# tensorflow/adanet

Measured on NVIDIA H100. Metric: candidate-train examples/sec per AdaNet iteration, higher is better.
Workload: dtype f32

## Files before the change

### adanet_b200/csrc/planes.cu

```cuda
#include <cuda.h>
#include <cudaTypedefs.h>

#include <stdlib.h>
#include <string.h>

#include <algorithm>
#include <atomic>
#include <mutex>
#include <string>
#include <unordered_map>
#include <vector>

#include "dense_simt.cuh"
#include "planes.cuh"
#include "wgmma.cuh"

namespace adn {
namespace pl {

static constexpr int BM = 128, BN = 64;
static constexpr int STAGES = 3;
static constexpr int A_TILE = BM * 128;
static constexpr int B_TILE = BN * 128;
static constexpr int STAGE_BYTES = 2 * A_TILE + 2 * B_TILE;
// ... 5 lines not shown
static_assert(128 * (PRODUCER_REGS + EPI_REGS) + 128 * CONSUMERS * CONSUMER_REGS <= 65536, "register file");
static_assert(PRODUCER_REGS < 65536 / NUM_THREADS && EPI_REGS > 65536 / NUM_THREADS &&
              CONSUMER_REGS > 65536 / NUM_THREADS, "setmaxnreg.dec / .inc");
static constexpr int ACC_BUFS = 2;
static constexpr int ACC_TILE_FLOATS = BM * BN;
static constexpr int ACC_BYTES = ACC_BUFS * ACC_TILE_FLOATS * 4;
static constexpr int EPI_STAGE_FLOATS = 32 * 16;
static constexpr int EPI_BYTES = EPI_WARPS * 2 * EPI_STAGE_FLOATS * 4;
static constexpr int BAR_BYTES = 256;
static constexpr int SMEM_BYTES = 1024 + STAGES * STAGE_BYTES + ACC_BYTES + EPI_BYTES + BAR_BYTES;
static_assert(SMEM_BYTES <= 232448, "shared memory per block");
static constexpr int MAX_SPLITS = 64;

template <int FMT> struct Fmt;
template <> struct Fmt<FMT_TF32> {
  static constexpr int BK = 32;
  static constexpr int CHUNK = 4;
};
template <> struct Fmt<FMT_F16> {
  static constexpr int BK = 64;
  static constexpr int CHUNK = 2;
};

enum { EPI_BIAS_ACT = 0, EPI_MASK = 1, EPI_PARTIAL = 2 };

struct GemmParams {
  int M, N;
  int tiles_m, tiles_n, splits;
  int tiles;
  float inv_tiles, inv_tiles_n, inv_tiles_m;
  int total_kb;
  int kb_per_split;
  int a_mn, b_mn;
  int out_planes;
  int m_fastest;
  void* out;
  void* out_lo;
  int ldc;
  int out_nb32;
  int out_tma;
  const float* bias;
  int act;
  uint32_t* out_bits;
  const uint32_t* mask_bits;
  float* colsum_part;
  int colsum_ld;
  float out_mul;
  unsigned int* ovf;
  uint32_t drop_thresh;
// ... 375 lines not shown
        }
        if (rsub == 0) {
          float* cp = g.colsum_part + (size_t)(mrow0 >> 5) * g.colsum_ld + col;
#pragma unroll
          for (int k = 0; k < 4; ++k)
            if (col + k < g.colsum_ld) cp[k] = cs[k];
        }
      }
    }
    __syncwarp();
  }
#undef ADN_SWZ
}

static constexpr int MAX_GROUP = 8;

struct alignas(64) Problem {
  CUtensorMap a_hi, a_lo, b_hi, b_lo;
  CUtensorMap o_hi, o_lo;
  GemmParams g;
  int item0;
  int pad_[3];
};
struct alignas(64) Group {
  Problem p[MAX_GROUP];
  int n;
  int total_items;
};

__device__ __forceinline__ int find_problem(const Group& grp, int cur, int item, int& next0) {
  while (item >= next0) {
    ++cur;
    next0 = (cur + 1 < grp.n) ? grp.p[cur + 1].item0 : 0x7fffffff;
  }
  return cur;
}
__device__ __forceinline__ int first_next0(const Group& grp) { return grp.n > 1 ? grp.p[1].item0 : 0x7fffffff; }

struct EpiItem {
  int p;
  Item it;
  uint32_t mw0, mw1;
  uint32_t drop_step;
};
template <int EPI>
__device__ __forceinline__ EpiItem epi_fetch(const Group& grp, int& cur, int& next0, int item, int tile_row) {
  EpiItem e;
  cur = find_problem(grp, cur, item, next0);
  e.p = cur;
  const GemmParams& g = grp.p[cur].g;
  e.it = decode_item(g, item - grp.p[cur].item0);
  e.mw0 = e.mw1 = 0xffffffffu;
  if (EPI == EPI_MASK && g.mask_bits) {
    const int my_row = e.it.m0 + tile_row, kbo = e.it.n0 >> 5;
    const bool row_ok = my_row < g.M;
    e.mw0 = (row_ok && kbo < g.out_nb32) ? __ldg(g.mask_bits + (size_t)kbo * g.M + my_row) : 0u;
    e.mw1 = (row_ok && kbo + 1 < g.out_nb32) ? __ldg(g.mask_bits + (size_t)(kbo + 1) * g.M + my_row) : 0u;
  }
  e.drop_step = (EPI == EPI_BIAS_ACT && g.drop_thresh != 0u) ? (uint32_t)(*g.drop_step) : 0u;
  return e;
}

template <int R> __device__ __forceinline__ void setmaxnreg_inc() { asm volatile("setmaxnreg.inc.sync.aligned.u32 %0;" ::"n"(R)); }
template <int R> __device__ __forceinline__ void setmaxnreg_dec() { asm volatile("setmaxnreg.dec.sync.aligned.u32 %0;" ::"n"(R)); }

__device__ __forceinline__ int acc_off(int row, int col) {
  return row * BN + ((((col >> 2) ^ row) & 7) | ((col >> 2) & 8)) * 4 + (col & 3);
}

template <int FMT>
__device__ __forceinline__ void fold_chunk(float (&acc)[32], const float (&H)[32], const float (&S)[32]) {
#pragma unroll
  for (int j = 0; j < 32; ++j) acc[j] += H[j];
  if (FMT == FMT_F16) {
#pragma unroll
    for (int j = 0; j < 32; ++j) acc[j] = fmaf(S[j], 1.0f / 2048.0f, acc[j]);
  } else {
#pragma unroll
    for (int j = 0; j < 32; ++j) acc[j] += S[j];
  }
}

template <int A_MN, int B_MN>
__device__ __forceinline__ void f16_kblock(uint32_t st, int wgi, float (&H)[32], float (&S)[32], bool first) {
  const uint32_t a_hi = st + (uint32_t)wgi * 8192u, a_lo = a_hi + A_TILE;
  const uint32_t b_hi = st + 2 * A_TILE, b_lo = b_hi + B_TILE;
  constexpr uint32_t a_step = A_MN ? 2048u : 32u, b_step = B_MN ? 2048u : 32u;
#pragma unroll
  for (int k = 0; k < 4; ++k) {
    const uint32_t sd = (first && k == 0) ? 0u : 1u;
    const uint64_t dah = wg::desc_sw128(a_hi + k * a_step), dal = wg::desc_sw128(a_lo + k * a_step);
    const uint64_t dbh = wg::desc_sw128(b_hi + k * b_step), dbl = wg::desc_sw128(b_lo + k * b_step);
    wg::mma_f16_n64<A_MN, B_MN>(H, dah, dbh, sd);
    wg::mma_f16_n64<A_MN, B_MN>(S, dah, dbl, sd);
    wg::mma_f16_n64<A_MN, B_MN>(S, dal, dbh, 1u);
  }
}

__device__ __forceinline__ uint32_t sw128_off(int r, int c) {
  return (uint32_t)(r * 128 + ((((c >> 4) ^ r) & 7) << 4) + (c & 15));
}
template <int MN>
// ... 13 lines not shown
  const uint8_t* bh = st + 2 * A_TILE;
  const uint8_t* bl = bh + B_TILE;
  const int gid = lane >> 2, tq = lane & 3;
#pragma unroll
  for (int ks = 0; ks < 4; ++ks) {
    uint32_t fa_h[4], fa_l[4];
#pragma unroll
    for (int e = 0; e < 4; ++e) {
      const uint32_t o = tf32_off<A_MN>(arow0 + gid + 8 * (e & 1), 8 * ks + tq + 4 * (e >> 1));
      fa_h[e] = *reinterpret_cast<const uint32_t*>(ah + o);
      fa_l[e] = *reinterpret_cast<const uint32_t*>(al + o);
    }
#pragma unroll
    for (int j = 0; j < 8; ++j) {
      const uint32_t o0 = tf32_off<B_MN>(8 * j + gid, 8 * ks + tq), o1 = tf32_off<B_MN>(8 * j + gid, 8 * ks + tq + 4);
      const uint32_t bh0 = *reinterpret_cast<const uint32_t*>(bh + o0), bh1 = *reinterpret_cast<const uint32_t*>(bh + o1);
      const uint32_t bl0 = *reinterpret_cast<const uint32_t*>(bl + o0), bl1 = *reinterpret_cast<const uint32_t*>(bl + o1);
      mma_tf32_16x8(&H[4 * j], fa_h, bh0, bh1);
      mma_tf32_16x8(&S[4 * j], fa_h, bl0, bl1);
      mma_tf32_16x8(&S[4 * j], fa_l, bh0, bh1);
    }
  }
}
template <int FMT, int EPI>
__global__ void __launch_bounds__(NUM_THREADS, 1)
pl_gemm_kernel(const __grid_constant__ Group grp) {
  constexpr int BK = Fmt<FMT>::BK;
  constexpr int CHUNK = Fmt<FMT>::CHUNK;
  constexpr int A_MN = EPI == EPI_PARTIAL, B_MN = EPI != EPI_MASK;
  extern __shared__ uint8_t smem_raw[];
  uint8_t* smem = reinterpret_cast<uint8_t*>((reinterpret_cast<uintptr_t>(smem_raw) + 1023) & ~(uintptr_t)1023);
  float* acc_stage = reinterpret_cast<float*>(smem + STAGES * STAGE_BYTES);
  float* epi_stage = reinterpret_cast<float*>(smem + STAGES * STAGE_BYTES + ACC_BYTES);
  uint64_t* bars = reinterpret_cast<uint64_t*>(smem + STAGES * STAGE_BYTES + ACC_BYTES + EPI_BYTES);
  uint64_t* full_bar = bars;
  uint64_t* empty_bar = bars + STAGES;
  uint64_t* tile_full = bars + 2 * STAGES;
  uint64_t* tile_empty = tile_full + ACC_BUFS;

  const int warp = __shfl_sync(0xffffffffu, threadIdx.x >> 5, 0);
  const int lane = threadIdx.x & 31;
  const int n_items = grp.total_items;

  if (threadIdx.x == 0) {
    for (int s = 0; s < STAGES; ++s) {
      mbar_init(smem_u32(&full_bar[s]), 1);
      mbar_init(smem_u32(&empty_bar[s]), CONSUMER_WARPS);
    }
    for (int b = 0; b < ACC_BUFS; ++b) {
      mbar_init(smem_u32(&tile_full[b]), 128 * CONSUMERS);
      mbar_init(smem_u32(&tile_empty[b]), 32 * EPI_WARPS);
    }
    asm volatile("fence.mbarrier_init.release.cluster;" ::: "memory");
  }
  if (warp == 1 && lane < grp.n) {
    tma_prefetch_desc(&grp.p[lane].a_hi);
    tma_prefetch_desc(&grp.p[lane].a_lo);
    tma_prefetch_desc(&grp.p[lane].b_hi);
    tma_prefetch_desc(&grp.p[lane].b_lo);
  }
  __syncthreads();

  if (warp < 4) {
    setmaxnreg_dec<PRODUCER_REGS>();
    if (warp == 0 && lane == 0) {
      uint32_t s = 0, ph = 0;
      int cur = 0, next0 = first_next0(grp);
      const uint32_t smem0 = smem_u32(smem);
      for (int item = blockIdx.x; item < n_items; item += gridDim.x) {
        cur = find_problem(grp, cur, item, next0);
        const Problem& pr = grp.p[cur];
        const GemmParams& g = pr.g;
        const Item it = decode_item(g, item - pr.item0);
        for (int kb = 0; kb < it.nkb; ++kb) {
          mbar_wait(smem_u32(&empty_bar[s]), ph ^ 1);
          const uint32_t fb = smem_u32(&full_bar[s]);
          mbar_expect_tx(fb, STAGE_BYTES);
          const uint32_t base = smem0 + s * STAGE_BYTES;
          const int kc = it.kb0 + kb;
          const int a1 = A_MN ? kc * BK : it.m0, a2 = A_MN ? (it.m0 / BK) : kc;
          const int b1 = B_MN ? kc * BK : it.n0, b2 = B_MN ? (it.n0 / BK) : kc;
          tma_load_3d(&pr.a_hi, fb, base, 0, a1, a2);
          tma_load_3d(&pr.a_lo, fb, base + A_TILE, 0, a1, a2);
          tma_load_3d(&pr.b_hi, fb, base + 2 * A_TILE, 0, b1, b2);
          tma_load_3d(&pr.b_lo, fb, base + 2 * A_TILE + B_TILE, 0, b1, b2);
          if (++s == STAGES) { s = 0; ph ^= 1; }
        }
      }
    }
    return;
  }

  if (warp >= 4 * (1 + CONSUMERS)) {
    setmaxnreg_inc<EPI_REGS>();
    const int ew = warp - 4 * (1 + CONSUMERS);
    float* stage = epi_stage + ew * 2 * EPI_STAGE_FLOATS;
    const int row = 32 * ew + lane;
    int cur = 0, next0 = first_next0(grp);
    EpiItem nx{};
    if ((int)blockIdx.x < n_items) nx = epi_fetch<EPI>(grp, cur, next0, blockIdx.x, row);
    uint32_t tcount = 0;
    for (int item = blockIdx.x; item < n_items; item += gridDim.x, ++tcount) {
      const EpiItem e = nx;
      if (item + (int)gridDim.x < n_items) nx = epi_fetch<EPI>(grp, cur, next0, item + gridDim.x, row);
      const GemmParams& g = grp.p[e.p].g;
      const Item& it = e.it;
      const uint32_t buf = tcount & 1u;
      mbar_wait(smem_u32(&tile_full[buf]), (tcount >> 1) & 1u);
      const float* tile = acc_stage + buf * ACC_TILE_FLOATS;
      const int mrow0 = it.m0 + 32 * ew;
      float* dense = reinterpret_cast<float*>(g.out);
      if (EPI == EPI_PARTIAL) dense += (size_t)it.split * g.M * g.N;
      const bool out_planes = g.out_planes != 0;
      const bool dense_vec = !out_planes && ((g.ldc & 3) == 0) && ((reinterpret_cast<uintptr_t>(dense) & 15) == 0);
      const int rows_ok = min(32, g.M - mrow0);
      const uint32_t mw0 = e.mw0, mw1 = e.mw1;
#pragma unroll 1
      for (int h = 0; h < 2; ++h) {
        const int cs = 32 * h;
        float acc[32];
#pragma unroll
        for (int q = 0; q < 8; ++q) {
          const float4 v = *reinterpret_cast<const float4*>(tile + acc_off(row, cs + 4 * q));
          acc[4 * q] = v.x; acc[4 * q + 1] = v.y; acc[4 * q + 2] = v.z; acc[4 * q + 3] = v.w;
        }
        if (h == 1) mbar_arrive(smem_u32(&tile_empty[buf]));
        const int ncol0 = it.n0 + cs;
        const uint32_t mw = h ? mw1 : mw0;
        if (FMT == FMT_F16 && !out_planes) {
          if (lane == 0) bulk_wait_read0();
          __syncwarp();
        }
        emit_slice<FMT, EPI>(g, out_planes, acc, mw, stage, lane, mrow0, ncol0, rows_ok, dense, dense_vec, true,
                             &grp.p[e.p].o_hi, &grp.p[e.p].o_lo, e.drop_step);
      }
    }
    if (FMT == FMT_F16 && lane == 0) bulk_wait0();
    return;
  }

  setmaxnreg_inc<CONSUMER_REGS>();
  const int wgi = warp / 4 - 1;
  const int wq = warp & 3;
  const int gid = lane >> 2, tq = lane & 3;
  const uint32_t smem0 = smem_u32(smem);
  uint32_t s = 0, ph = 0;
  int cur = 0, next0 = first_next0(grp);
  uint32_t tcount = 0;
  float H[32], S[32];
#pragma unroll
  for (int j = 0; j < 32; ++j) H[j] = S[j] = 0.f;
  for (int item = blockIdx.x; item < n_items; item += gridDim.x, ++tcount) {
    cur = find_problem(grp, cur, item, next0);
    const GemmParams& g = grp.p[cur].g;
    const Item it = decode_item(g, item - grp.p[cur].item0);
    float acc[32];
#pragma unroll
    for (int j = 0; j < 8; ++j)
#pragma unroll
      for (int e = 0; e < 4; ++e) {
        const int col = it.n0 + 8 * j + 2 * tq + (e & 1);
        acc[4 * j + e] = (EPI == EPI_BIAS_ACT && g.bias && col < g.N) ? __ldg(g.bias + col) : 0.f;
      }
    for (int kb = 0; kb < it.nkb; ++kb) {
      const bool first = (kb % CHUNK) == 0;
      const bool last = (kb % CHUNK) == CHUNK - 1 || kb == it.nkb - 1;
      mbar_wait(smem_u32(&full_bar[s]), ph);
      if (FMT == FMT_F16) {
        wg::fence_regs(H);
        wg::fence_regs(S);
        wg::fence();
        f16_kblock<A_MN, B_MN>(smem0 + s * STAGE_BYTES, wgi, H, S, first);
        wg::commit();
        wg::wait<0>();
        wg::fence_regs(H);
        wg::fence_regs(S);
      } else {
        if (first) {
#pragma unroll
          for (int j = 0; j < 32; ++j) H[j] = S[j] = 0.f;
        }
        tf32_kblock<A_MN, B_MN>(smem + s * STAGE_BYTES, 64 * wgi + 16 * wq, lane, H, S);
      }
      __syncwarp();
      if (lane == 0) mbar_arrive(smem_u32(&empty_bar[s]));
      if (++s == STAGES) { s = 0; ph ^= 1; }
      if (last) fold_chunk<FMT>(acc, H, S);
    }
    const uint32_t buf = tcount & 1u;
    mbar_wait(smem_u32(&tile_empty[buf]), ((tcount >> 1) & 1u) ^ 1u);
    float* tile = acc_stage + buf * ACC_TILE_FLOATS;
#pragma unroll
    for (int j = 0; j < 8; ++j) {
      const int row = 64 * wgi + 16 * wq + gid, col = 8 * j + 2 * tq;
      *reinterpret_cast<float2*>(tile + acc_off(row, col)) = make_float2(acc[4 * j], acc[4 * j + 1]);
      *reinterpret_cast<float2*>(tile + acc_off(row + 8, col)) = make_float2(acc[4 * j + 2], acc[4 * j + 3]);
    }
    mbar_arrive(smem_u32(&tile_full[buf]));
  }
}

template <int FMT>
__global__ void __launch_bounds__(256)
split_kernel(const float* __restrict__ src, void* __restrict__ hi_, void* __restrict__ lo_, uint32_t* __restrict__ bits,
             int rows, int cols, int nkb, float scale, unsigned int* ovf) {
  constexpr int BK = Fmt<FMT>::BK;
  const int vec_per_row = nkb * (BK / 4);
  const int64_t nvec = (int64_t)rows * vec_per_row;
  const int64_t nvec_pad = (nvec + 31) & ~(int64_t)31;
  const bool vec_src = ((cols & 3) == 0) && ((reinterpret_cast<uintptr_t>(src) & 15) == 0);
  bool over = false;
  for (int64_t i = (int64_t)blockIdx.x * blockDim.x + threadIdx.x; i < nvec_pad; i += (int64_t)gridDim.x * blockDim.x) {
    const bool live = i < nvec;
    const int r = live ? (int)(i / vec_per_row) : 0;
    const int c = live ? (int)(i % vec_per_row) * 4 : 0;
    float v[4] = {0.f, 0.f, 0.f, 0.f};
    if (live) {
      if (vec_src && c + 3 < cols) {
        float4 t = __ldg(reinterpret_cast<const float4*>(src + (size_t)r * cols + c));
        v[0] = t.x; v[1] = t.y; v[2] = t.z; v[3] = t.w;
      } else {
// ... 82 lines not shown
  ADN_CUDA(cudaStreamSynchronize(st));
  *out_host = (int)v;
  return ADN_OK;
}

int init() {
  static std::once_flag once;
  static int rc = ADN_OK;
  std::call_once(once, []() {
    void* fn = nullptr;
    cudaDriverEntryPointQueryResult q;
    cudaError_t e = cudaGetDriverEntryPoint("cuTensorMapEncodeTiled", &fn, cudaEnableDefault, &q);
    if (e != cudaSuccess || q != cudaDriverEntryPointSuccess || fn == nullptr) {
      (void)cudaGetLastError();
      rc = fail(ADN_ERR_CUDA, "pl::init: cuTensorMapEncodeTiled entry point unavailable");
      return;
    }
    g_encode = reinterpret_cast<PFN_cuTensorMapEncodeTiled>(fn);
    bool ok = true;
#define ADN_PL_ATTR(F, E) \
  ok = ok && (cudaFuncSetAttribute(pl_gemm_kernel<F, E>, cudaFuncAttributeMaxDynamicSharedMemorySize, SMEM_BYTES) == cudaSuccess)
    ADN_PL_ATTR(FMT_TF32, EPI_BIAS_ACT); ADN_PL_ATTR(FMT_TF32, EPI_MASK); ADN_PL_ATTR(FMT_TF32, EPI_PARTIAL);
    ADN_PL_ATTR(FMT_F16, EPI_BIAS_ACT); ADN_PL_ATTR(FMT_F16, EPI_MASK); ADN_PL_ATTR(FMT_F16, EPI_PARTIAL);
#undef ADN_PL_ATTR
    if (!ok) {
      (void)cudaGetLastError();
      rc = fail(ADN_ERR_CUDA, "pl::init: cudaFuncSetAttribute(smem=%d) failed", SMEM_BYTES);
      return;
    }
    void* addr = nullptr;
    if (cudaGetSymbolAddress(&addr, g_plane_overflow) != cudaSuccess || !addr) {
      (void)cudaGetLastError();
      rc = fail(ADN_ERR_CUDA, "pl::init: cudaGetSymbolAddress(g_plane_overflow) failed");
      return;
    }
    g_ovf_addr = reinterpret_cast<unsigned int*>(addr);
  });
  return rc;
}

int64_t planes_bytes_fmt(int fmt, int64_t rows, int64_t cols) { return planes_bytes(fmt, rows, cols); }

struct Operand {
  const void* hi;
  const void* lo;
  int64_t rows, nkb;
// ... 95 lines not shown
  GemmParams g;
};

static int encode_maps(int fmt, const GemmDesc& d, CUtensorMap* a_hi, CUtensorMap* a_lo, CUtensorMap* b_hi, CUtensorMap* b_lo,
                       const char* what) {
  if ((reinterpret_cast<uintptr_t>(d.a.hi) | reinterpret_cast<uintptr_t>(d.a.lo) | reinterpret_cast<uintptr_t>(d.b.hi) |
       reinterpret_cast<uintptr_t>(d.b.lo)) & 127)
    return fail(ADN_ERR_INVALID, "%s: plane buffers must be 256 B aligned", what);
  int rc;
  if ((rc = make_map(fmt, a_hi, d.a.hi, d.a.rows, d.a.nkb, d.a.mn_major, BM))) return rc;
  if ((rc = make_map(fmt, a_lo, d.a.lo, d.a.rows, d.a.nkb, d.a.mn_major, BM))) return rc;
  if ((rc = make_map(fmt, b_hi, d.b.hi, d.b.rows, d.b.nkb, d.b.mn_major, BN))) return rc;
  if ((rc = make_map(fmt, b_lo, d.b.lo, d.b.rows, d.b.nkb, d.b.mn_major, BN))) return rc;
  return ADN_OK;
}

static int item_order_m_fastest(const GemmParams& g) {
  static const int env = getenv("ADN_PL_MFAST") ? atoi(getenv("ADN_PL_MFAST")) : -1;
  if (env >= 0) return env;
  (void)g;
  return 0;
}

template <int FMT, int EPI>
static void launch_kernel(const Group& grp, int grid, cudaStream_t st) {
  pl_gemm_kernel<FMT, EPI><<<grid, NUM_THREADS, SMEM_BYTES, st>>>(grp);
}
template <int EPI>
static int launch_group(int fmt, const GemmDesc* d, int n, cudaStream_t st, const char* what) {
  {
    for (int i0 = 0; i0 < n; i0 += MAX_GROUP) {
      const int m = std::min(MAX_GROUP, n - i0);
      Group grp;
      memset(&grp, 0, sizeof(grp));
      int items = 0;
      for (int i = 0; i < m; ++i) {
        const GemmDesc& src = d[i0 + i];
        Problem& pr = grp.p[i];
        if (src.a.mn_major != (EPI == EPI_PARTIAL) || src.b.mn_major != (EPI != EPI_MASK))
          return fail(ADN_ERR_INVALID, "%s: operand majorness does not match the epilogue kind", what);
        int rc = encode_maps(fmt, src, &pr.a_hi, &pr.a_lo, &pr.b_hi, &pr.b_lo, what);
        if (rc) return rc;
        pr.g = src.g;
        pr.g.out_tma = 0;
        if (fmt == FMT_F16 && EPI != EPI_PARTIAL && src.g.out_planes && store_mode() && (src.g.out_nb32 & 1) == 0 &&
            ((reinterpret_cast<uintptr_t>(src.g.out) | reinterpret_cast<uintptr_t>(src.g.out_lo)) & 127) == 0) {
          if ((rc = make_store_map(&pr.o_hi, src.g.out, src.g.M, src.g.out_nb32 / 2))) return rc;
          if ((rc = make_store_map(&pr.o_lo, src.g.out_lo, src.g.M, src.g.out_nb32 / 2))) return rc;
          pr.g.out_tma = 1;
        }
        pr.g.a_mn = src.a.mn_major;
        pr.g.b_mn = src.b.mn_major;
        pr.g.tiles_m = (int)ceil_div(pr.g.M, BM);
        pr.g.tiles_n = (int)ceil_div(pr.g.N, BN);
        pr.g.tiles = pr.g.tiles_m * pr.g.tiles_n;
        if ((int64_t)pr.g.tiles * pr.g.splits >= (1 << 21))
          return fail(ADN_ERR_UNSUPPORTED, "%s: %d work items exceed the decode range", what, pr.g.tiles * pr.g.splits);
        pr.g.inv_tiles = 1.0f / (float)pr.g.tiles;
        pr.g.inv_tiles_n = 1.0f / (float)pr.g.tiles_n;
        pr.g.inv_tiles_m = 1.0f / (float)pr.g.tiles_m;
        pr.g.m_fastest = item_order_m_fastest(pr.g);
        pr.g.ovf = g_ovf_addr;
        pr.item0 = items;
        items += pr.g.tiles_m * pr.g.tiles_n * pr.g.splits;
      }
      grp.n = m;
      grp.total_items = items;
      const int grid = std::min(items, sm_count());
      if (fmt == FMT_F16) launch_kernel<FMT_F16, EPI>(grp, grid, st);
      else launch_kernel<FMT_TF32, EPI>(grp, grid, st);
      ADN_CHECK_LAUNCH(what);
    }
  }
  return ADN_OK;
}

int split(int fmt, const float* src, int64_t rows, int64_t cols, void* planes, int log2_scale, cudaStream_t st) {
  const int bk = fmt_bk(fmt);
  const int64_t nkb = ceil_div(cols, bk);
  const int64_t nvec = rows * nkb * (bk / 4);
  const int blocks = (int)std::max<int64_t>(1, std::min<int64_t>(ceil_div(nvec, 256), (int64_t)sm_count() * 16));
  const PlaneView v = plane_view(fmt, planes, rows, cols);
  const float scale = ldexpf(1.0f, log2_scale);
  if (fmt == FMT_F16)
    split_kernel<FMT_F16><<<blocks, 256, 0, st>>>(src, v.hi, v.lo, v.bits, (int)rows, (int)cols, (int)nkb, scale, g_ovf_addr);
  else
    split_kernel<FMT_TF32><<<blocks, 256, 0, st>>>(src, v.hi, v.lo, v.bits, (int)rows, (int)cols, (int)nkb, scale, g_ovf_addr);
  ADN_CHECK_LAUNCH("planes split");
  return ADN_OK;
}

int merge(int fmt, const void* planes, int64_t rows, int64_t cols, float* dst, cudaStream_t st) {
  const int bk = fmt_bk(fmt);
  const int64_t nkb = ceil_div(cols, bk);
  const int64_t n = rows * nkb * bk;
  const int blocks = (int)std::max<int64_t>(1, std::min<int64_t>(ceil_div(n, 256), (int64_t)sm_count() * 16));
// ... 144 lines not shown
      GemmDesc e;
      e.a = operand(fmt, o.dzp, batch, o.out, 0);
      e.b = operand(fmt, o.wp, o.in, o.out, 0);
      GemmParams g{};
      g.M = (int)batch; g.N = (int)o.in;
      g.total_kb = (int)ceil_div(o.out, bk); g.kb_per_split = g.total_kb; g.splits = 1;
      g.mask_bits = o.x_relu_mask ? bits_of(fmt, o.xp, batch, o.in) : nullptr;
      g.out_nb32 = (int)bits_blocks(fmt, o.in);
      g.colsum_part = o.dx_colsum ? c.cspart : nullptr;
      g.colsum_ld = (int)o.in;
      if (o.dxp) {
        const PlaneView v = plane_view(fmt, o.dxp, batch, o.in);
        g.out_planes = 1;
        g.out = v.hi; g.out_lo = v.lo;
        g.out_mul = o.dx_mul;
      } else {
        g.out = o.dx; g.ldc = (int)o.in;
        g.out_mul = unscale * o.dx_mul;
      }
      e.g = g;
      dxd.push_back(e);
    }
  }
  int rc;
  if (!dwd.empty()) {
    if ((rc = launch_group<EPI_PARTIAL>(fmt, dwd.data(), (int)dwd.size(), st, "pl dW gemm"))) return rc;
    std::vector<simt::ReduceJob> jobs;
    for (int i = 0; i < n; ++i)
      if (ops[i].dw && cv[(size_t)i].splits > 1)
        jobs.push_back(simt::ReduceJob{cv[(size_t)i].part, ops[i].dw, ops[i].in * ops[i].out, cv[(size_t)i].splits,
                                       ops[i].in * ops[i].out, ldexpf(1.0f, -ops[i].dz_log2_scale)});
    if ((rc = simt::reduce_partials_group(jobs.data(), (int)jobs.size(), st))) return rc;
  }
  if (!dxd.empty()) {
    if ((rc = launch_group<EPI_MASK>(fmt, dxd.data(), (int)dxd.size(), st, "pl dX gemm"))) return rc;
    std::vector<simt::ColsumJob> jobs;
    for (int i = 0; i < n; ++i)
      if (ops[i].dx_colsum && (ops[i].dxp || ops[i].dx))
        jobs.push_back(simt::ColsumJob{cv[(size_t)i].cspart, ops[i].dx_colsum, ceil_div(batch, 32), ops[i].in,
                                       cv[(size_t)i].cspart2, ops[i].dxp ? ldexpf(1.0f, -ops[i].dz_log2_scale) : 1.0f});
    if ((rc = simt::colsum_group(jobs.data(), (int)jobs.size(), st))) return rc;
  }
  return ADN_OK;
}

int dense_fwd(int fmt, const void* xp, const void* wp, const float* bias, void* yp, float* y, int64_t batch, int64_t in,
              int64_t out, int act, cudaStream_t st) {
  FwdOp op{xp, wp, bias, yp, y, in, out, act};
  return dense_fwd_group(fmt, &op, 1, batch, st);
}

int dense_bwd(int fmt, const void* xp, const void* wp, const void* dzp, void* dxp, float* dx, float* dx_colsum, float* dw,
              int64_t batch, int64_t in, int64_t out, int x_relu_mask, int dz_log2_scale, void* ws, int64_t ws_bytes,
              cudaStream_t st) {
  BwdOp op{xp, wp, dzp, dxp, dx, dx_colsum, dw, in, out, x_relu_mask, dz_log2_scale, ws, ws_bytes};
  return dense_bwd_group(fmt, &op, 1, batch, st);
}

}
}
```

Measured before the change: 9.392 million.

## Fuse backward dW and dX GEMMs into one mixed persistent kernel launch

Adds an EPI_MIXED kernel variant that runs the dX (masked) and dW (split-partial) backward GEMMs in a single persistent launch. Each CTA interleaves short dX tiles with chunked dW k-block steps using a credit-based walk, so the two GEMMs share the SMs and each epilogue type is chosen per tile. The aim is to remove one kernel launch and the tail and underfill of two separate small grouped GEMMs. In exchange the parameter block is larger and the scheduling is more complex. The path is used only when dX has at most one chunk of k and both groups fit, and it can be turned off with an environment variable.

```diff
diff --git a/adanet_b200/csrc/planes.cu b/adanet_b200/csrc/planes.cu
--- a/adanet_b200/csrc/planes.cu
+++ b/adanet_b200/csrc/planes.cu
@@ -51,9 +51,10 @@
   static constexpr int CHUNK = 2;
 };
 
-enum { EPI_BIAS_ACT = 0, EPI_MASK = 1, EPI_PARTIAL = 2 };
+enum { EPI_BIAS_ACT = 0, EPI_MASK = 1, EPI_PARTIAL = 2, EPI_MIXED = 3 };
 
 struct GemmParams {
+  int epi;
   int M, N;
   int tiles_m, tiles_n, splits;
   int tiles;
@@ -475,20 +476,102 @@
   int item0;
   int pad_[3];
 };
-struct alignas(64) Group {
-  Problem p[MAX_GROUP];
+template <int CAP>
+struct alignas(64) GroupT {
+  Problem p[CAP];
   int n;
   int total_items;
+  int x_items;
+  int x_q, x_r;
 };
-
-__device__ __forceinline__ int find_problem(const Group& grp, int cur, int item, int& next0) {
+using Group = GroupT<MAX_GROUP>;
+using MixGroup = GroupT<2 * MAX_GROUP>;
+template <int EPI> using GroupOf = GroupT<EPI == EPI_MIXED ? 2 * MAX_GROUP : MAX_GROUP>;
+static_assert(sizeof(MixGroup) <= 32764, "kernel parameter limit");
+
+template <class G>
+__device__ __forceinline__ int find_problem(const G& grp, int cur, int item, int& next0) {
   while (item >= next0) {
     ++cur;
     next0 = (cur + 1 < grp.n) ? grp.p[cur + 1].item0 : 0x7fffffff;
   }
   return cur;
 }
-__device__ __forceinline__ int first_next0(const Group& grp) { return grp.n > 1 ? grp.p[1].item0 : 0x7fffffff; }
+template <class G>
+__device__ __forceinline__ int first_next0(const G& grp) { return grp.n > 1 ? grp.p[1].item0 : 0x7fffffff; }
+
+struct MixStep {
+  int p;
+  Item it;
+  bool dw;
+  bool first;
+  bool tile;
+  int kb_begin, kb_end;
+};
+template <int STEP>
+struct MixWalk {
+  int xi, wi;
+  int nx, nw;
+  int xleft, wleft, credit;
+  int wc;
+  int curx, nextx, curw, nextw;
+
+  static __device__ __forceinline__ int steps(int nkb) { return STEP ? (nkb + STEP - 1) / STEP : 1; }
+  template <class G>
+  __device__ __forceinline__ void init(const G& grp) {
+    const int c = blockIdx.x, grid = gridDim.x;
+    xi = c;
+    wi = grp.x_items + (grid - 1 - c);
+    nx = grp.x_q + (c < grp.x_r ? 1 : 0);
+    nw = 0;
+    int cur = 0, next0 = first_next0(grp);
+    for (int item = wi; item < grp.total_items; item += grid) {
+      cur = find_problem(grp, cur, item, next0);
+      nw += steps(decode_item(grp.p[cur].g, item - grp.p[cur].item0).nkb);
+    }
+    xleft = nx;
+    wleft = nw;
+    credit = 0;
+    wc = 0;
+    curx = curw = 0;
+    nextx = nextw = first_next0(grp);
+  }
+  template <class G>
+  __device__ __forceinline__ bool next(const G& grp, MixStep& s) {
+    if (xleft > 0 && (wleft == 0 || credit < nx)) {
+      curx = find_problem(grp, curx, xi, nextx);
+      s.p = curx;
+      s.it = decode_item(grp.p[curx].g, xi - grp.p[curx].item0);
+      s.dw = false;
+      s.first = s.tile = true;
+      s.kb_begin = 0;
+      s.kb_end = s.it.nkb;
+      xi += gridDim.x;
+      --xleft;
+      credit += nw;
+      return true;
+    }
+    if (wleft > 0) {
+      curw = find_problem(grp, curw, wi, nextw);
+      s.p = curw;
+      s.it = decode_item(grp.p[curw].g, wi - grp.p[curw].item0);
+      const int nch = steps(s.it.nkb);
+      s.dw = true;
+      s.first = wc == 0;
+      s.tile = wc == nch - 1;
+      s.kb_begin = wc * STEP;
+      s.kb_end = STEP ? min(s.it.nkb, s.kb_begin + STEP) : s.it.nkb;
+      if (++wc == nch) {
+        wc = 0;
+        wi += gridDim.x;
+      }
+      --wleft;
+      credit -= nx;
+      return true;
+    }
+    return false;
+  }
+};
 
 struct EpiItem {
   int p;
@@ -497,20 +580,24 @@
   uint32_t drop_step;
 };
 template <int EPI>
+__device__ __forceinline__ void epi_words(const GemmParams& g, EpiItem& e, int tile_row) {
+  e.mw0 = e.mw1 = 0xffffffffu;
+  if (EPI == EPI_MASK && g.mask_bits) {
+    const int my_row = e.it.m0 + tile_row, kbo = e.it.n0 >> 5;
+    const bool row_ok = my_row < g.M;
+    e.mw0 = (row_ok && kbo < g.out_nb32) ? __ldg(g.mask_bits + (size_t)kbo * g.M + my_row) : 0u;
+    e.mw1 = (row_ok && kbo + 1 < g.out_nb32) ? __ldg(g.mask_bits + (size_t)(kbo + 1) * g.M + my_row) : 0u;
+  }
+  e.drop_step = (EPI == EPI_BIAS_ACT && g.drop_thresh != 0u) ? (uint32_t)(*g.drop_step) : 0u;
+}
+template <int EPI>
 __device__ __forceinline__ EpiItem epi_fetch(const Group& grp, int& cur, int& next0, int item, int tile_row) {
   EpiItem e;
   cur = find_problem(grp, cur, item, next0);
   e.p = cur;
   const GemmParams& g = grp.p[cur].g;
   e.it = decode_item(g, item - grp.p[cur].item0);
-  e.mw0 = e.mw1 = 0xffffffffu;
-  if (EPI == EPI_MASK && g.mask_bits) {
-    const int my_row = e.it.m0 + tile_row, kbo = e.it.n0 >> 5;
-    const bool row_ok = my_row < g.M;
-    e.mw0 = (row_ok && kbo < g.out_nb32) ? __ldg(g.mask_bits + (size_t)kbo * g.M + my_row) : 0u;
-    e.mw1 = (row_ok && kbo + 1 < g.out_nb32) ? __ldg(g.mask_bits + (size_t)(kbo + 1) * g.M + my_row) : 0u;
-  }
-  e.drop_step = (EPI == EPI_BIAS_ACT && g.drop_thresh != 0u) ? (uint32_t)(*g.drop_step) : 0u;
+  epi_words<EPI>(g, e, tile_row);
   return e;
 }
 
@@ -531,6 +618,19 @@
   } else {
 #pragma unroll
     for (int j = 0; j < 32; ++j) acc[j] += S[j];
+  }
+}
+
+template <int FMT>
+__device__ __forceinline__ void fold_fresh(float (&H)[32], const float (&S)[32]) {
+#pragma unroll
+  for (int j = 0; j < 32; ++j) H[j] = 0.f + H[j];
+  if (FMT == FMT_F16) {
+#pragma unroll
+    for (int j = 0; j < 32; ++j) H[j] = fmaf(S[j], 1.0f / 2048.0f, H[j]);
+  } else {
+#pragma unroll
+    for (int j = 0; j < 32; ++j) H[j] += S[j];
   }
 }
 
@@ -590,12 +690,118 @@
     }
   }
 }
+
+template <int BK>
+__device__ __forceinline__ void produce_kblocks(const Problem& pr, const Item& it, int kb_begin, int kb_end, int a_mn, int b_mn,
+                                                uint32_t smem0, uint64_t* full_bar, uint64_t* empty_bar, uint32_t& s,
+                                                uint32_t& ph) {
+  for (int kb = kb_begin; kb < kb_end; ++kb) {
+    mbar_wait(smem_u32(&empty_bar[s]), ph ^ 1);
+    const uint32_t fb = smem_u32(&full_bar[s]);
+    mbar_expect_tx(fb, STAGE_BYTES);
+    const uint32_t base = smem0 + s * STAGE_BYTES;
+    const int kc = it.kb0 + kb;
+    const int a1 = a_mn ? kc * BK : it.m0, a2 = a_mn ? (it.m0 / BK) : kc;
+    const int b1 = b_mn ? kc * BK : it.n0, b2 = b_mn ? (it.n0 / BK) : kc;
+    tma_load_3d(&pr.a_hi, fb, base, 0, a1, a2);
+    tma_load_3d(&pr.a_lo, fb, base + A_TILE, 0, a1, a2);
+    tma_load_3d(&pr.b_hi, fb, base + 2 * A_TILE, 0, b1, b2);
+    tma_load_3d(&pr.b_lo, fb, base + 2 * A_TILE + B_TILE, 0, b1, b2);
+    if (++s == STAGES) { s = 0; ph ^= 1; }
+  }
+}
+
+template <int FMT, int A_MN, int B_MN, bool FRESH = false>
+__device__ __forceinline__ void consume_kblocks(uint8_t* smem, int wgi, int wq, int lane, uint64_t* full_bar,
+                                                uint64_t* empty_bar, uint32_t& s, uint32_t& ph, int kb_begin, int kb_end,
+                                                int nkb, float (&acc)[32], float (&H)[32], float (&S)[32]) {
+  constexpr int CHUNK = Fmt<FMT>::CHUNK;
+  const uint32_t smem0 = smem_u32(smem);
+  for (int kb = kb_begin; kb < kb_end; ++kb) {
+    const bool first = (kb % CHUNK) == 0;
+    const bool last = (kb % CHUNK) == CHUNK - 1 || kb == nkb - 1;
+    mbar_wait(smem_u32(&full_bar[s]), ph);
+    if (FMT == FMT_F16) {
+      wg::fence_regs(H);
+      wg::fence_regs(S);
+      wg::fence();
+      f16_kblock<A_MN, B_MN>(smem0 + s * STAGE_BYTES, wgi, H, S, first);
+      wg::commit();
+      wg::wait<0>();
+      wg::fence_regs(H);
+      wg::fence_regs(S);
+    } else {
+      if (first) {
+#pragma unroll
+        for (int j = 0; j < 32; ++j) H[j] = S[j] = 0.f;
+      }
+      tf32_kblock<A_MN, B_MN>(smem + s * STAGE_BYTES, 64 * wgi + 16 * wq, lane, H, S);
+    }
+    __syncwarp();
+    if (lane == 0) mbar_arrive(smem_u32(&empty_bar[s]));
+    if (++s == STAGES) { s = 0; ph ^= 1; }
+    if (last) {
+      if (FRESH) fold_fresh<FMT>(H, S);
+      else fold_chunk<FMT>(acc, H, S);
+    }
+  }
+}
+
+__device__ __forceinline__ void stage_tile(float* acc_stage, uint64_t* tile_full, uint64_t* tile_empty, uint32_t tcount,
+                                           int wgi, int wq, int lane, const float (&acc)[32]) {
+  const int gid = lane >> 2, tq = lane & 3;
+  const uint32_t buf = tcount & 1u;
+  mbar_wait(smem_u32(&tile_empty[buf]), ((tcount >> 1) & 1u) ^ 1u);
+  float* tile = acc_stage + buf * ACC_TILE_FLOATS;
+#pragma unroll
+  for (int j = 0; j < 8; ++j) {
+    const int row = 64 * wgi + 16 * wq + gid, col = 8 * j + 2 * tq;
+    *reinterpret_cast<float2*>(tile + acc_off(row, col)) = make_float2(acc[4 * j], acc[4 * j + 1]);
+    *reinterpret_cast<float2*>(tile + acc_off(row + 8, col)) = make_float2(acc[4 * j + 2], acc[4 * j + 3]);
+  }
+  mbar_arrive(smem_u32(&tile_full[buf]));
+}
+
+template <int FMT, int EPI>
+__device__ __forceinline__ void epi_tile(const Problem& pr, const EpiItem& e, const float* tile, uint32_t empty_bar,
+                                         float* stage, int ew, int lane, int row) {
+  const GemmParams& g = pr.g;
+  const Item& it = e.it;
+  const int mrow0 = it.m0 + 32 * ew;
+  float* dense = reinterpret_cast<float*>(g.out);
+  if (EPI == EPI_PARTIAL) dense += (size_t)it.split * g.M * g.N;
+  const bool out_planes = g.out_planes != 0;
+  const bool dense_vec = !out_planes && ((g.ldc & 3) == 0) && ((reinterpret_cast<uintptr_t>(dense) & 15) == 0);
+  const int rows_ok = min(32, g.M - mrow0);
+  const uint32_t mw0 = e.mw0, mw1 = e.mw1;
+#pragma unroll 1
+  for (int h = 0; h < 2; ++h) {
+    const int cs = 32 * h;
+    float acc[32];
+#pragma unroll
+    for (int q = 0; q < 8; ++q) {
+      const float4 v = *reinterpret_cast<const float4*>(tile + acc_off(row, cs + 4 * q));
+      acc[4 * q] = v.x; acc[4 * q + 1] = v.y; acc[4 * q + 2] = v.z; acc[4 * q + 3] = v.w;
+    }
+    if (h == 1) mbar_arrive(empty_bar);
+    const int ncol0 = it.n0 + cs;
+    const uint32_t mw = h ? mw1 : mw0;
+    if (FMT == FMT_F16 && !out_planes) {
+      if (lane == 0) bulk_wait_read0();
+      __syncwarp();
+    }
+    emit_slice<FMT, EPI>(g, out_planes, acc, mw, stage, lane, mrow0, ncol0, rows_ok, dense, dense_vec, true, &pr.o_hi,
+                         &pr.o_lo, e.drop_step);
+  }
+}
+
 template <int FMT, int EPI>
 __global__ void __launch_bounds__(NUM_THREADS, 1)
-pl_gemm_kernel(const __grid_constant__ Group grp) {
+pl_gemm_kernel(const __grid_constant__ GroupOf<EPI> grp) {
   constexpr int BK = Fmt<FMT>::BK;
   constexpr int CHUNK = Fmt<FMT>::CHUNK;
   constexpr int A_MN = EPI == EPI_PARTIAL, B_MN = EPI != EPI_MASK;
+  constexpr int MIX_STEP = FMT == FMT_F16 ? CHUNK : 0;
   extern __shared__ uint8_t smem_raw[];
   uint8_t* smem = reinterpret_cast<uint8_t*>((reinterpret_cast<uintptr_t>(smem_raw) + 1023) & ~(uintptr_t)1023);
   float* acc_stage = reinterpret_cast<float*>(smem + STAGES * STAGE_BYTES);
@@ -633,26 +839,22 @@
     setmaxnreg_dec<PRODUCER_REGS>();
     if (warp == 0 && lane == 0) {
       uint32_t s = 0, ph = 0;
-      int cur = 0, next0 = first_next0(grp);
       const uint32_t smem0 = smem_u32(smem);
-      for (int item = blockIdx.x; item < n_items; item += gridDim.x) {
-        cur = find_problem(grp, cur, item, next0);
-        const Problem& pr = grp.p[cur];
-        const GemmParams& g = pr.g;
-        const Item it = decode_item(g, item - pr.item0);
-        for (int kb = 0; kb < it.nkb; ++kb) {
-          mbar_wait(smem_u32(&empty_bar[s]), ph ^ 1);
-          const uint32_t fb = smem_u32(&full_bar[s]);
-          mbar_expect_tx(fb, STAGE_BYTES);
-          const uint32_t base = smem0 + s * STAGE_BYTES;
-          const int kc = it.kb0 + kb;
-          const int a1 = A_MN ? kc * BK : it.m0, a2 = A_MN ? (it.m0 / BK) : kc;
-          const int b1 = B_MN ? kc * BK : it.n0, b2 = B_MN ? (it.n0 / BK) : kc;
-          tma_load_3d(&pr.a_hi, fb, base, 0, a1, a2);
-          tma_load_3d(&pr.a_lo, fb, base + A_TILE, 0, a1, a2);
-          tma_load_3d(&pr.b_hi, fb, base + 2 * A_TILE, 0, b1, b2);
-          tma_load_3d(&pr.b_lo, fb, base + 2 * A_TILE + B_TILE, 0, b1, b2);
-          if (++s == STAGES) { s = 0; ph ^= 1; }
+      if constexpr (EPI == EPI_MIXED) {
+        MixWalk<MIX_STEP> w;
+        w.init(grp);
+        MixStep st;
+        while (w.next(grp, st)) {
+          const Problem& pr = grp.p[st.p];
+          produce_kblocks<BK>(pr, st.it, st.kb_begin, st.kb_end, pr.g.a_mn, pr.g.b_mn, smem0, full_bar, empty_bar, s, ph);
+        }
+      } else {
+        int cur = 0, next0 = first_next0(grp);
+        for (int item = blockIdx.x; item < n_items; item += gridDim.x) {
+          cur = find_problem(grp, cur, item, next0);
+          const Problem& pr = grp.p[cur];
+          const Item it = decode_item(pr.g, item - pr.item0);
+          produce_kblocks<BK>(pr, it, 0, it.nkb, A_MN, B_MN, smem0, full_bar, empty_bar, s, ph);
         }
       }
     }
@@ -664,43 +866,49 @@
     const int ew = warp - 4 * (1 + CONSUMERS);
     float* stage = epi_stage + ew * 2 * EPI_STAGE_FLOATS;
     const int row = 32 * ew + lane;
-    int cur = 0, next0 = first_next0(grp);
-    EpiItem nx{};
-    if ((int)blockIdx.x < n_items) nx = epi_fetch<EPI>(grp, cur, next0, blockIdx.x, row);
-    uint32_t tcount = 0;
-    for (int item = blockIdx.x; item < n_items; item += gridDim.x, ++tcount) {
-      const EpiItem e = nx;
-      if (item + (int)gridDim.x < n_items) nx = epi_fetch<EPI>(grp, cur, next0, item + gridDim.x, row);
-      const GemmParams& g = grp.p[e.p].g;
-      const Item& it = e.it;
-      const uint32_t buf = tcount & 1u;
-      mbar_wait(smem_u32(&tile_full[buf]), (tcount >> 1) & 1u);
-      const float* tile = acc_stage + buf * ACC_TILE_FLOATS;
-      const int mrow0 = it.m0 + 32 * ew;
-      float* dense = reinterpret_cast<float*>(g.out);
-      if (EPI == EPI_PARTIAL) dense += (size_t)it.split * g.M * g.N;
-      const bool out_planes = g.out_planes != 0;
-      const bool dense_vec = !out_planes && ((g.ldc & 3) == 0) && ((reinterpret_cast<uintptr_t>(dense) & 15) == 0);
-      const int rows_ok = min(32, g.M - mrow0);
-      const uint32_t mw0 = e.mw0, mw1 = e.mw1;
-#pragma unroll 1
-      for (int h = 0; h < 2; ++h) {
-        const int cs = 32 * h;
-        float acc[32];
-#pragma unroll
-        for (int q = 0; q < 8; ++q) {
-          const float4 v = *reinterpret_cast<const float4*>(tile + acc_off(row, cs + 4 * q));
-          acc[4 * q] = v.x; acc[4 * q + 1] = v.y; acc[4 * q + 2] = v.z; acc[4 * q + 3] = v.w;
-        }
-        if (h == 1) mbar_arrive(smem_u32(&tile_empty[buf]));
-        const int ncol0 = it.n0 + cs;
-        const uint32_t mw = h ? mw1 : mw0;
-        if (FMT == FMT_F16 && !out_planes) {
-          if (lane == 0) bulk_wait_read0();
-          __syncwarp();
-        }
-        emit_slice<FMT, EPI>(g, out_planes, acc, mw, stage, lane, mrow0, ncol0, rows_ok, dense, dense_vec, true,
-                             &grp.p[e.p].o_hi, &grp.p[e.p].o_lo, e.drop_step);
+    if constexpr (EPI == EPI_MIXED) {
+      MixWalk<MIX_STEP> w;
+      w.init(grp);
+      MixStep ns;
+      auto next_tile = [&]() {
+        while (w.next(grp, ns))
+          if (ns.tile) return true;
+        return false;
+      };
+      auto fetch = [&]() {
+        EpiItem e;
+        e.p = ns.p;
+        e.it = ns.it;
+        if (ns.dw) epi_words<EPI_PARTIAL>(grp.p[ns.p].g, e, row);
+        else epi_words<EPI_MASK>(grp.p[ns.p].g, e, row);
+        return e;
+      };
+      bool have = next_tile();
+      EpiItem nx{};
+      bool nx_dw = false;
+      if (have) { nx = fetch(); nx_dw = ns.dw; }
+      for (uint32_t tcount = 0; have; ++tcount) {
+        const EpiItem e = nx;
+        const bool dw = nx_dw;
+        have = next_tile();
+        if (have) { nx = fetch(); nx_dw = ns.dw; }
+        const uint32_t buf = tcount & 1u;
+        mbar_wait(smem_u32(&tile_full[buf]), (tcount >> 1) & 1u);
+        const float* tile = acc_stage + buf * ACC_TILE_FLOATS;
+        if (dw) epi_tile<FMT, EPI_PARTIAL>(grp.p[e.p], e, tile, smem_u32(&tile_empty[buf]), stage, ew, lane, row);
+        else epi_tile<FMT, EPI_MASK>(grp.p[e.p], e, tile, smem_u32(&tile_empty[buf]), stage, ew, lane, row);
+      }
+    } else {
+      int cur = 0, next0 = first_next0(grp);
+      EpiItem nx{};
+      if ((int)blockIdx.x < n_items) nx = epi_fetch<EPI>(grp, cur, next0, blockIdx.x, row);
+      uint32_t tcount = 0;
+      for (int item = blockIdx.x; item < n_items; item += gridDim.x, ++tcount) {
+        const EpiItem e = nx;
+        if (item + (int)gridDim.x < n_items) nx = epi_fetch<EPI>(grp, cur, next0, item + gridDim.x, row);
+        const uint32_t buf = tcount & 1u;
+        mbar_wait(smem_u32(&tile_full[buf]), (tcount >> 1) & 1u);
+        epi_tile<FMT, EPI>(grp.p[e.p], e, acc_stage + buf * ACC_TILE_FLOATS, smem_u32(&tile_empty[buf]), stage, ew, lane, row);
       }
     }
     if (FMT == FMT_F16 && lane == 0) bulk_wait0();
@@ -710,61 +918,62 @@
   setmaxnreg_inc<CONSUMER_REGS>();
   const int wgi = warp / 4 - 1;
   const int wq = warp & 3;
-  const int gid = lane >> 2, tq = lane & 3;
-  const uint32_t smem0 = smem_u32(smem);
   uint32_t s = 0, ph = 0;
-  int cur = 0, next0 = first_next0(grp);
   uint32_t tcount = 0;
   float H[32], S[32];
 #pragma unroll
   for (int j = 0; j < 32; ++j) H[j] = S[j] = 0.f;
-  for (int item = blockIdx.x; item < n_items; item += gridDim.x, ++tcount) {
-    cur = find_problem(grp, cur, item, next0);
-    const GemmParams& g = grp.p[cur].g;
-    const Item it = decode_item(g, item - grp.p[cur].item0);
-    float acc[32];
-#pragma unroll
-    for (int j = 0; j < 8; ++j)
-#pragma unroll
-      for (int e = 0; e < 4; ++e) {
-        const int col = it.n0 + 8 * j + 2 * tq + (e & 1);
-        acc[4 * j + e] = (EPI == EPI_BIAS_ACT && g.bias && col < g.N) ? __ldg(g.bias + col) : 0.f;
+  if constexpr (EPI == EPI_MIXED) {
+    MixWalk<MIX_STEP> w;
+    w.init(grp);
+    MixStep st;
+    float accw[32];
+#pragma unroll
+    for (int j = 0; j < 32; ++j) accw[j] = 0.f;
+    while (w.next(grp, st)) {
+      if (st.dw) {
+        if (MIX_STEP == 0) {
+          float acc[32];
+#pragma unroll
+          for (int j = 0; j < 32; ++j) acc[j] = 0.f;
+          consume_kblocks<FMT, 1, 1>(smem, wgi, wq, lane, full_bar, empty_bar, s, ph, 0, st.it.nkb, st.it.nkb, acc, H, S);
+#pragma unroll
+          for (int j = 0; j < 32; ++j) H[j] = acc[j];
+        } else {
+          if (st.first) {
+#pragma unroll
+            for (int j = 0; j < 32; ++j) accw[j] = 0.f;
+          }
+          consume_kblocks<FMT, 1, 1>(smem, wgi, wq, lane, full_bar, empty_bar, s, ph, st.kb_begin, st.kb_end, st.it.nkb,
+                                     accw, H, S);
+          if (!st.tile) continue;
+#pragma unroll
+          for (int j = 0; j < 32; ++j) H[j] = accw[j];
+        }
+      } else {
+        consume_kblocks<FMT, 0, 0, true>(smem, wgi, wq, lane, full_bar, empty_bar, s, ph, 0, st.it.nkb, st.it.nkb, H, H,
+                                         S);
       }
-    for (int kb = 0; kb < it.nkb; ++kb) {
-      const bool first = (kb % CHUNK) == 0;
-      const bool last = (kb % CHUNK) == CHUNK - 1 || kb == it.nkb - 1;
-      mbar_wait(smem_u32(&full_bar[s]), ph);
-      if (FMT == FMT_F16) {
-        wg::fence_regs(H);
-        wg::fence_regs(S);
-        wg::fence();
-        f16_kblock<A_MN, B_MN>(smem0 + s * STAGE_BYTES, wgi, H, S, first);
-        wg::commit();
-        wg::wait<0>();
-        wg::fence_regs(H);
-        wg::fence_regs(S);
-      } else {
-        if (first) {
-#pragma unroll
-          for (int j = 0; j < 32; ++j) H[j] = S[j] = 0.f;
+      stage_tile(acc_stage, tile_full, tile_empty, tcount++, wgi, wq, lane, H);
+    }
+  } else {
+    const int tq = lane & 3;
+    int cur = 0, next0 = first_next0(grp);
+    for (int item = blockIdx.x; item < n_items; item += gridDim.x, ++tcount) {
+      cur = find_problem(grp, cur, item, next0);
+      const GemmParams& g = grp.p[cur].g;
+      const Item it = decode_item(g, item - grp.p[cur].item0);
+      float acc[32];
+#pragma unroll
+      for (int j = 0; j < 8; ++j)
+#pragma unroll
+        for (int e = 0; e < 4; ++e) {
+          const int col = it.n0 + 8 * j + 2 * tq + (e & 1);
+          acc[4 * j + e] = (EPI == EPI_BIAS_ACT && g.bias && col < g.N) ? __ldg(g.bias + col) : 0.f;
         }
-        tf32_kblock<A_MN, B_MN>(smem + s * STAGE_BYTES, 64 * wgi + 16 * wq, lane, H, S);
-      }
-      __syncwarp();
-      if (lane == 0) mbar_arrive(smem_u32(&empty_bar[s]));
-      if (++s == STAGES) { s = 0; ph ^= 1; }
-      if (last) fold_chunk<FMT>(acc, H, S);
-    }
-    const uint32_t buf = tcount & 1u;
-    mbar_wait(smem_u32(&tile_empty[buf]), ((tcount >> 1) & 1u) ^ 1u);
-    float* tile = acc_stage + buf * ACC_TILE_FLOATS;
-#pragma unroll
-    for (int j = 0; j < 8; ++j) {
-      const int row = 64 * wgi + 16 * wq + gid, col = 8 * j + 2 * tq;
-      *reinterpret_cast<float2*>(tile + acc_off(row, col)) = make_float2(acc[4 * j], acc[4 * j + 1]);
-      *reinterpret_cast<float2*>(tile + acc_off(row + 8, col)) = make_float2(acc[4 * j + 2], acc[4 * j + 3]);
-    }
-    mbar_arrive(smem_u32(&tile_full[buf]));
+      consume_kblocks<FMT, A_MN, B_MN>(smem, wgi, wq, lane, full_bar, empty_bar, s, ph, 0, it.nkb, it.nkb, acc, H, S);
+      stage_tile(acc_stage, tile_full, tile_empty, tcount, wgi, wq, lane, acc);
+    }
   }
 }
 
@@ -893,6 +1102,7 @@
   ok = ok && (cudaFuncSetAttribute(pl_gemm_kernel<F, E>, cudaFuncAttributeMaxDynamicSharedMemorySize, SMEM_BYTES) == cudaSuccess)
     ADN_PL_ATTR(FMT_TF32, EPI_BIAS_ACT); ADN_PL_ATTR(FMT_TF32, EPI_MASK); ADN_PL_ATTR(FMT_TF32, EPI_PARTIAL);
     ADN_PL_ATTR(FMT_F16, EPI_BIAS_ACT); ADN_PL_ATTR(FMT_F16, EPI_MASK); ADN_PL_ATTR(FMT_F16, EPI_PARTIAL);
+    ADN_PL_ATTR(FMT_TF32, EPI_MIXED); ADN_PL_ATTR(FMT_F16, EPI_MIXED);
 #undef ADN_PL_ATTR
     if (!ok) {
       (void)cudaGetLastError();
@@ -1034,56 +1244,86 @@
   return 0;
 }
 
+static int bwd_mix_mode() {
+  static const int env = getenv("ADN_PL_BWD_MIX") ? atoi(getenv("ADN_PL_BWD_MIX")) : 1;
+  return env;
+}
+
 template <int FMT, int EPI>
-static void launch_kernel(const Group& grp, int grid, cudaStream_t st) {
+static void launch_kernel(const GroupOf<EPI>& grp, int grid, cudaStream_t st) {
   pl_gemm_kernel<FMT, EPI><<<grid, NUM_THREADS, SMEM_BYTES, st>>>(grp);
 }
+
+static int setup_problem(int fmt, int epi, const GemmDesc& src, Problem& pr, int& items, const char* what) {
+  if (src.a.mn_major != (epi == EPI_PARTIAL) || src.b.mn_major != (epi != EPI_MASK))
+    return fail(ADN_ERR_INVALID, "%s: operand majorness does not match the epilogue kind", what);
+  int rc = encode_maps(fmt, src, &pr.a_hi, &pr.a_lo, &pr.b_hi, &pr.b_lo, what);
+  if (rc) return rc;
+  pr.g = src.g;
+  pr.g.epi = epi;
+  pr.g.out_tma = 0;
+  if (fmt == FMT_F16 && epi != EPI_PARTIAL && src.g.out_planes && store_mode() && (src.g.out_nb32 & 1) == 0 &&
+      ((reinterpret_cast<uintptr_t>(src.g.out) | reinterpret_cast<uintptr_t>(src.g.out_lo)) & 127) == 0) {
+    if ((rc = make_store_map(&pr.o_hi, src.g.out, src.g.M, src.g.out_nb32 / 2))) return rc;
+    if ((rc = make_store_map(&pr.o_lo, src.g.out_lo, src.g.M, src.g.out_nb32 / 2))) return rc;
+    pr.g.out_tma = 1;
+  }
+  pr.g.a_mn = src.a.mn_major;
+  pr.g.b_mn = src.b.mn_major;
+  pr.g.tiles_m = (int)ceil_div(pr.g.M, BM);
+  pr.g.tiles_n = (int)ceil_div(pr.g.N, BN);
+  pr.g.tiles = pr.g.tiles_m * pr.g.tiles_n;
+  if ((int64_t)pr.g.tiles * pr.g.splits >= (1 << 21))
+    return fail(ADN_ERR_UNSUPPORTED, "%s: %d work items exceed the decode range", what, pr.g.tiles * pr.g.splits);
+  pr.g.inv_tiles = 1.0f / (float)pr.g.tiles;
+  pr.g.inv_tiles_n = 1.0f / (float)pr.g.tiles_n;
+  pr.g.inv_tiles_m = 1.0f / (float)pr.g.tiles_m;
+  pr.g.m_fastest = item_order_m_fastest(pr.g);
+  pr.g.ovf = g_ovf_addr;
+  pr.item0 = items;
+  items += pr.g.tiles_m * pr.g.tiles_n * pr.g.splits;
+  return ADN_OK;
+}
+
 template <int EPI>
 static int launch_group(int fmt, const GemmDesc* d, int n, cudaStream_t st, const char* what) {
-  {
-    for (int i0 = 0; i0 < n; i0 += MAX_GROUP) {
-      const int m = std::min(MAX_GROUP, n - i0);
-      Group grp;
-      memset(&grp, 0, sizeof(grp));
-      int items = 0;
-      for (int i = 0; i < m; ++i) {
-        const GemmDesc& src = d[i0 + i];
-        Problem& pr = grp.p[i];
-        if (src.a.mn_major != (EPI == EPI_PARTIAL) || src.b.mn_major != (EPI != EPI_MASK))
-          return fail(ADN_ERR_INVALID, "%s: operand majorness does not match the epilogue kind", what);
-        int rc = encode_maps(fmt, src, &pr.a_hi, &pr.a_lo, &pr.b_hi, &pr.b_lo, what);
-        if (rc) return rc;
-        pr.g = src.g;
-        pr.g.out_tma = 0;
-        if (fmt == FMT_F16 && EPI != EPI_PARTIAL && src.g.out_planes && store_mode() && (src.g.out_nb32 & 1) == 0 &&
-            ((reinterpret_cast<uintptr_t>(src.g.out) | reinterpret_cast<uintptr_t>(src.g.out_lo)) & 127) == 0) {
-          if ((rc = make_store_map(&pr.o_hi, src.g.out, src.g.M, src.g.out_nb32 / 2))) return rc;
-          if ((rc = make_store_map(&pr.o_lo, src.g.out_lo, src.g.M, src.g.out_nb32 / 2))) return rc;
-          pr.g.out_tma = 1;
-        }
-        pr.g.a_mn = src.a.mn_major;
-        pr.g.b_mn = src.b.mn_major;
-        pr.g.tiles_m = (int)ceil_div(pr.g.M, BM);
-        pr.g.tiles_n = (int)ceil_div(pr.g.N, BN);
-        pr.g.tiles = pr.g.tiles_m * pr.g.tiles_n;
-        if ((int64_t)pr.g.tiles * pr.g.splits >= (1 << 21))
-          return fail(ADN_ERR_UNSUPPORTED, "%s: %d work items exceed the decode range", what, pr.g.tiles * pr.g.splits);
-        pr.g.inv_tiles = 1.0f / (float)pr.g.tiles;
-        pr.g.inv_tiles_n = 1.0f / (float)pr.g.tiles_n;
-        pr.g.inv_tiles_m = 1.0f / (float)pr.g.tiles_m;
-        pr.g.m_fastest = item_order_m_fastest(pr.g);
-        pr.g.ovf = g_ovf_addr;
-        pr.item0 = items;
-        items += pr.g.tiles_m * pr.g.tiles_n * pr.g.splits;
-      }
-      grp.n = m;
-      grp.total_items = items;
-      const int grid = std::min(items, sm_count());
-      if (fmt == FMT_F16) launch_kernel<FMT_F16, EPI>(grp, grid, st);
-      else launch_kernel<FMT_TF32, EPI>(grp, grid, st);
-      ADN_CHECK_LAUNCH(what);
-    }
-  }
+  for (int i0 = 0; i0 < n; i0 += MAX_GROUP) {
+    const int m = std::min(MAX_GROUP, n - i0);
+    Group grp;
+    memset(&grp, 0, sizeof(grp));
+    int items = 0;
+    for (int i = 0; i < m; ++i) {
+      const int rc = setup_problem(fmt, EPI, d[i0 + i], grp.p[i], items, what);
+      if (rc) return rc;
+    }
+    grp.n = m;
+    grp.total_items = items;
+    const int grid = std::min(items, sm_count());
+    if (fmt == FMT_F16) launch_kernel<FMT_F16, EPI>(grp, grid, st);
+    else launch_kernel<FMT_TF32, EPI>(grp, grid, st);
+    ADN_CHECK_LAUNCH(what);
+  }
+  return ADN_OK;
+}
+
+static int launch_mixed(int fmt, const GemmDesc* dx, int nx, const GemmDesc* dw, int nw, cudaStream_t st) {
+  const char* what = "pl dW+dX gemm";
+  MixGroup grp;
+  memset(&grp, 0, sizeof(grp));
+  int items = 0, rc;
+  for (int i = 0; i < nx; ++i)
+    if ((rc = setup_problem(fmt, EPI_MASK, dx[i], grp.p[i], items, what))) return rc;
+  grp.x_items = items;
+  for (int i = 0; i < nw; ++i)
+    if ((rc = setup_problem(fmt, EPI_PARTIAL, dw[i], grp.p[nx + i], items, what))) return rc;
+  grp.n = nx + nw;
+  grp.total_items = items;
+  const int grid = std::min(items, sm_count());
+  grp.x_q = grp.x_items / grid;
+  grp.x_r = grp.x_items % grid;
+  if (fmt == FMT_F16) launch_kernel<FMT_F16, EPI_MIXED>(grp, grid, st);
+  else launch_kernel<FMT_TF32, EPI_MIXED>(grp, grid, st);
+  ADN_CHECK_LAUNCH(what);
   return ADN_OK;
 }
 
@@ -1274,24 +1514,39 @@
       dxd.push_back(e);
     }
   }
-  int rc;
-  if (!dwd.empty()) {
-    if ((rc = launch_group<EPI_PARTIAL>(fmt, dwd.data(), (int)dwd.size(), st, "pl dW gemm"))) return rc;
+  const int chunk = fmt == FMT_F16 ? Fmt<FMT_F16>::CHUNK : Fmt<FMT_TF32>::CHUNK;
+  bool mixed = bwd_mix_mode() && !dwd.empty() && !dxd.empty() && dwd.size() <= (size_t)MAX_GROUP &&
+               dxd.size() <= (size_t)MAX_GROUP;
+  for (const GemmDesc& e : dxd) mixed = mixed && e.g.total_kb <= chunk;
+  auto reduce_dw = [&]() {
     std::vector<simt::ReduceJob> jobs;
     for (int i = 0; i < n; ++i)
       if (ops[i].dw && cv[(size_t)i].splits > 1)
         jobs.push_back(simt::ReduceJob{cv[(size_t)i].part, ops[i].dw, ops[i].in * ops[i].out, cv[(size_t)i].splits,
                                        ops[i].in * ops[i].out, ldexpf(1.0f, -ops[i].dz_log2_scale)});
-    if ((rc = simt::reduce_partials_group(jobs.data(), (int)jobs.size(), st))) return rc;
-  }
-  if (!dxd.empty()) {
-    if ((rc = launch_group<EPI_MASK>(fmt, dxd.data(), (int)dxd.size(), st, "pl dX gemm"))) return rc;
+    return simt::reduce_partials_group(jobs.data(), (int)jobs.size(), st);
+  };
+  auto colsum_dx = [&]() {
     std::vector<simt::ColsumJob> jobs;
     for (int i = 0; i < n; ++i)
       if (ops[i].dx_colsum && (ops[i].dxp || ops[i].dx))
         jobs.push_back(simt::ColsumJob{cv[(size_t)i].cspart, ops[i].dx_colsum, ceil_div(batch, 32), ops[i].in,
                                        cv[(size_t)i].cspart2, ops[i].dxp ? ldexpf(1.0f, -ops[i].dz_log2_scale) : 1.0f});
-    if ((rc = simt::colsum_group(jobs.data(), (int)jobs.size(), st))) return rc;
+    return simt::colsum_group(jobs.data(), (int)jobs.size(), st);
+  };
+  int rc;
+  if (mixed) {
+    if ((rc = launch_mixed(fmt, dxd.data(), (int)dxd.size(), dwd.data(), (int)dwd.size(), st))) return rc;
+    if ((rc = reduce_dw())) return rc;
+    return colsum_dx();
+  }
+  if (!dwd.empty()) {
+    if ((rc = launch_group<EPI_PARTIAL>(fmt, dwd.data(), (int)dwd.size(), st, "pl dW gemm"))) return rc;
+    if ((rc = reduce_dw())) return rc;
+  }
+  if (!dxd.empty()) {
+    if ((rc = launch_group<EPI_MASK>(fmt, dxd.data(), (int)dxd.size(), st, "pl dX gemm"))) return rc;
+    if ((rc = colsum_dx())) return rc;
   }
   return ADN_OK;
 }
```

After: 9.591 million, median of 6. 1.02x the previous value.
